# ray-project/ray_shuffling_data_loader

Hardware: AMD Instinct MI355X
Metric: shuffled_rows_per_sec (higher is better)
Workload: dtype bf16; 1 GPU; model=shuffling-data-loader + TabularMLP(100-512-256-128-1), global_batch=250000, rows_per_gpu=12500000, num_cols=100, batch_size_per_rank=250000, num_reducers=4, max_concurrent_epochs=2, parallelism=dp1, seed=0, burn_steps=0

## Files before the change

csrc/shuffle_kernels.hip:

```cpp

#include <hip/hip_runtime.h>
#include <hip/hip_fp16.h>
#include <hip/hip_bf16.h>

#include <cstdint>

#define RSDL_MAX_COLS 128

namespace rsdl {

__global__ void gather_rows_u4_kernel(
    const uint4* __restrict__ src,
    uint4* __restrict__ dst,
    const int64_t* __restrict__ perm,
    int64_t n_rows,
    int64_t row_u4) {
  const int64_t total = n_rows * row_u4;
  const int64_t stride = (int64_t)gridDim.x * blockDim.x;
  for (int64_t i = (int64_t)blockIdx.x * blockDim.x + threadIdx.x; i < total;
       i += stride) {
    const int64_t row = i / row_u4;
    const int64_t j = i - row * row_u4;
    dst[i] = src[perm[row] * row_u4 + j];
  }
// ... 28 lines not shown

struct ColDesc {
  int64_t col_ptr;
  int32_t packed_off;
  int32_t src_dtype;
  int32_t dst_dtype;
  int32_t numel;
};

struct ColTable {
  ColDesc cols[RSDL_MAX_COLS];
};

template <typename S, typename D>
__device__ __forceinline__ D cast_elem(S v) {
  return (D)v;
}
template <>
__device__ __forceinline__ __hip_bfloat16 cast_elem(float v) {
  return __float2bfloat16(v);
}
template <>
__device__ __forceinline__ __hip_bfloat16 cast_elem(double v) {
  return __float2bfloat16((float)v);
}
template <>
__device__ __forceinline__ __hip_bfloat16 cast_elem(int32_t v) {
  return __float2bfloat16((float)v);
}
template <>
__device__ __forceinline__ __hip_bfloat16 cast_elem(int64_t v) {
  return __float2bfloat16((float)v);
}
template <>
__device__ __forceinline__ float cast_elem(__hip_bfloat16 v) {
  return __bfloat162float(v);
}
template <>
__device__ __forceinline__ double cast_elem(__hip_bfloat16 v) {
  return (double)__bfloat162float(v);
}

__device__ __forceinline__ void unpack_vec4_f32_f32(
    const uint8_t* __restrict__ packed, int64_t row_stride,
    const int64_t* __restrict__ perm, float* __restrict__ dst,
    int32_t packed_off, int32_t numel, int64_t n_rows, int64_t tid,
    int64_t nthreads) {
// ... 57 lines not shown
}

template <typename S, typename D>
__device__ void pack_col_loop(
    uint8_t* __restrict__ packed,
    int64_t row_stride,
    const int64_t* __restrict__ perm,
    const S* __restrict__ src,
    int32_t packed_off,
    int32_t numel,
    int64_t n_rows,
    int64_t tid,
    int64_t nthreads) {
  const int64_t total = n_rows * numel;
  for (int64_t i = tid; i < total; i += nthreads) {
    const int64_t row = i / numel;
    const int64_t e = i - row * numel;
    const int64_t drow = perm ? perm[row] : row;
    D* dp = reinterpret_cast<D*>(packed + drow * row_stride + packed_off);
    dp[e] = cast_elem<S, D>(src[i]);
  }
}

#define RSDL_DISPATCH_DST(S_CTYPE, SRC_DT, DST_DT, CALL)                   \
  switch (DST_DT) {                                                        \
    case DT_F32: { using D = float; CALL; break; }                         \
    case DT_F64: { using D = double; CALL; break; }                        \
    case DT_I32: { using D = int32_t; CALL; break; }                       \
    case DT_I64: { using D = int64_t; CALL; break; }                       \
    case DT_BF16: { using D = __hip_bfloat16; CALL; break; }               \
    default: break;                                                        \
  }

#define RSDL_DISPATCH_PAIR(SRC_DT, DST_DT, CALL)                           \
  switch (SRC_DT) {                                                        \
    case DT_F32: { using S = float; RSDL_DISPATCH_DST(float, SRC_DT,       \
                   DST_DT, CALL); break; }                                 \
    case DT_F64: { using S = double; RSDL_DISPATCH_DST(double, SRC_DT,     \
                   DST_DT, CALL); break; }                                 \
    case DT_I32: { using S = int32_t; RSDL_DISPATCH_DST(int32_t, SRC_DT,   \
                   DST_DT, CALL); break; }                                 \
    case DT_I64: { using S = int64_t; RSDL_DISPATCH_DST(int64_t, SRC_DT,   \
                   DST_DT, CALL); break; }                                 \
    default: break;                                                        \
  }

// ... 4 lines not shown
    ColTable table,
    int32_t num_cols,
    int64_t n_rows) {
  const int32_t c = blockIdx.y;
  if (c >= num_cols) return;
  const ColDesc d = table.cols[c];
  const int64_t tid = (int64_t)blockIdx.x * blockDim.x + threadIdx.x;
  const int64_t nthreads = (int64_t)gridDim.x * blockDim.x;
  if (d.src_dtype == DT_F32 && (d.numel & 3) == 0 &&
      (d.packed_off & 15) == 0) {
    if (d.dst_dtype == DT_F32) {
      unpack_vec4_f32_f32(packed, row_stride, perm,
                          reinterpret_cast<float*>(d.col_ptr), d.packed_off,
                          d.numel, n_rows, tid, nthreads);
      return;
    }
    if (d.dst_dtype == DT_BF16) {
      unpack_vec4_f32_bf16(packed, row_stride, perm,
                           reinterpret_cast<__hip_bfloat16*>(d.col_ptr),
                           d.packed_off, d.numel, n_rows, tid, nthreads);
      return;
    }
  }
  RSDL_DISPATCH_PAIR(
      d.src_dtype, d.dst_dtype,
      (unpack_col_loop<S, D>(packed, row_stride, perm,
                             reinterpret_cast<D*>(d.col_ptr), d.packed_off,
                             d.numel, n_rows, tid, nthreads)));
}

__global__ void pack_columns_kernel(
    uint8_t* __restrict__ packed,
    int64_t row_stride,
    const int64_t* __restrict__ perm,
    ColTable table,
    int32_t num_cols,
    int64_t n_rows) {
  const int32_t c = blockIdx.y;
  if (c >= num_cols) return;
  const ColDesc d = table.cols[c];
  const int64_t tid = (int64_t)blockIdx.x * blockDim.x + threadIdx.x;
  const int64_t nthreads = (int64_t)gridDim.x * blockDim.x;
  RSDL_DISPATCH_PAIR(
      d.dst_dtype, d.src_dtype,
      (pack_col_loop<S, D>(packed, row_stride, perm,
                           reinterpret_cast<const S*>(d.col_ptr),
                           d.packed_off, d.numel, n_rows, tid, nthreads)));
}


#define RSDL_PART_MAX_DESTS 1024
// ... 523 lines not shown
  const ColDesc d = table.cols[c];
  const int64_t tid = (int64_t)blockIdx.x * blockDim.x + threadIdx.x;
  const int64_t nthreads = (int64_t)gridDim.x * blockDim.x;
  const bool al16 =
      ((reinterpret_cast<uintptr_t>(packed) + (uintptr_t)d.packed_off) &
       15) == 0;
  const int32_t ab = abase.base[c];
  if (ab < 0) {
    if (d.src_dtype == DT_F32 && (d.numel & 3) == 0 &&
        (d.packed_off & 15) == 0) {
      if (d.dst_dtype == DT_F32) {
        unpack_vec4_f32_f32(packed, row_stride, perm,
                            reinterpret_cast<float*>(d.col_ptr),
                            d.packed_off, d.numel, n_rows, tid, nthreads);
        return;
      }
      if (d.dst_dtype == DT_BF16) {
        unpack_vec4_f32_bf16(packed, row_stride, perm,
                             reinterpret_cast<__hip_bfloat16*>(d.col_ptr),
                             d.packed_off, d.numel, n_rows, tid, nthreads);
        return;
      }
    }
    RSDL_DISPATCH_PAIR(
        d.src_dtype, d.dst_dtype,
        (unpack_col_loop<S, D>(packed, row_stride, perm,
                               reinterpret_cast<D*>(d.col_ptr),
                               d.packed_off, d.numel, n_rows, tid,
                               nthreads)));
    return;
  }
  const double2* aff = aff_table + ab;
  const bool fill = has_fill != 0;
  const bool vec_dst = d.dst_dtype == DT_F32 || d.dst_dtype == DT_BF16;
  if (vec_dst && (d.numel & 3) == 0 && d.src_dtype == DT_F64) {
    if (d.dst_dtype == DT_BF16) {
      __hip_bfloat16* o = reinterpret_cast<__hip_bfloat16*>(d.col_ptr);
      if (al16)
        unpack_affine_vec4_f64<__hip_bfloat16, true>(
            packed, row_stride, perm, o, aff, d.packed_off, d.numel, n_rows,
            tid, nthreads, fill, fill_f);
      else
        unpack_affine_vec4_f64<__hip_bfloat16, false>(
            packed, row_stride, perm, o, aff, d.packed_off, d.numel, n_rows,
            tid, nthreads, fill, fill_f);
    } else {
// ... 9 lines not shown
    }
    return;
  }
  if (vec_dst && (d.numel & 3) == 0 && d.src_dtype == DT_F32 && al16) {
    if (d.dst_dtype == DT_BF16)
      unpack_affine_vec4_f32<__hip_bfloat16>(
          packed, row_stride, perm,
          reinterpret_cast<__hip_bfloat16*>(d.col_ptr), aff, d.packed_off,
          d.numel, n_rows, tid, nthreads, fill, fill_f);
    else
      unpack_affine_vec4_f32<float>(
          packed, row_stride, perm, reinterpret_cast<float*>(d.col_ptr),
          aff, d.packed_off, d.numel, n_rows, tid, nthreads, fill, fill_f);
    return;
  }
  RSDL_DISPATCH_PAIR(
      d.src_dtype, d.dst_dtype,
      (unpack_affine_col_loop<S, D>(packed, row_stride, perm,
                                    reinterpret_cast<D*>(d.col_ptr), aff,
                                    d.packed_off, d.numel, n_rows, tid,
                                    nthreads, fill, fill_f)));
}

void launch_column_stats(
    const void* packed, int64_t row_stride, int64_t n_rows,
    const StatsTable& table, int32_t num_cols, int32_t total_elems,
    int32_t num_blocks, int64_t* part_n, double* part_s, double* part_ss,
    double* pivot, int64_t* out_n, double* out_s, double* out_ss,
    hipStream_t stream) {
  hipLaunchKernelGGL(column_stats_kernel, dim3(num_blocks),
                     dim3(RSDL_STATS_THREADS), 0, stream,
                     reinterpret_cast<const uint8_t*>(packed), row_stride,
                     n_rows, table, num_cols, total_elems, part_n, part_s,
                     part_ss, pivot);
  const int threads = 64;
  hipLaunchKernelGGL(column_stats_combine_kernel,
                     dim3((total_elems + threads - 1) / threads),
                     dim3(threads), 0, stream, part_n, part_s, part_ss,
                     num_blocks, total_elems, out_n, out_s, out_ss);
}

void launch_unpack_permute_affine(
    const void* packed, int64_t row_stride, const int64_t* perm,
    const ColTable& table, const AffineBase& abase, const void* aff_table,
    int32_t num_cols, int64_t n_rows, int32_t has_fill, float fill_f,
    hipStream_t stream) {
// ... 14 lines not shown
```

csrc/shuffle_ops.cpp:

```cpp

#include <torch/extension.h>

#include <c10/hip/HIPStream.h>
#include <hip/hip_runtime.h>

#include <cmath>
#include <cstdlib>
#include <cstring>
#include <tuple>
#include <vector>

#include "chain.h"
#include "step_glue.h"

namespace rsdl {

enum DType : int32_t {
  DT_F32 = 0,
  DT_F64 = 1,
  DT_I32 = 2,
  DT_I64 = 3,
  DT_F16 = 4,
  DT_BF16 = 5,
  DT_U8 = 6,
// ... 30 lines not shown
  int32_t elem_base;
};

struct StatsTable {
  StatsCol cols[128];
};

struct AffineBase {
  int32_t base[128];
};

void launch_column_stats(const void* packed, int64_t row_stride,
                         int64_t n_rows, const StatsTable& table,
                         int32_t num_cols, int32_t total_elems,
                         int32_t num_blocks, int64_t* part_n, double* part_s,
                         double* part_ss, double* pivot, int64_t* out_n,
                         double* out_s, double* out_ss, hipStream_t stream);
void launch_unpack_permute_affine(const void* packed, int64_t row_stride,
                                  const int64_t* perm, const ColTable& table,
                                  const AffineBase& abase,
                                  const void* aff_table, int32_t num_cols,
                                  int64_t n_rows, int32_t has_fill,
                                  float fill_f, hipStream_t stream);
void launch_partition_hist(const int32_t* dest, int32_t* block_counts,
                           int64_t n, int32_t num_dests, int32_t num_blocks,
                           hipStream_t stream);
void launch_partition_scatter(const int32_t* dest, const int32_t* block_base,
                              int32_t* perm_out, int64_t n, int32_t num_dests,
                              int32_t num_blocks, hipStream_t stream);
void launch_pack_tiled(void* packed, int64_t row_stride, const ColTable& table,
                       int32_t num_cols, int64_t n_rows, int32_t tile_rows,
                       int64_t lds_bytes, int32_t n8, hipStream_t stream);
void launch_wgrad_bf16(const void* dy, const void* x, float* dW, float* db,
                       int64_t M, int32_t N, int32_t K, int32_t split_m,
                       hipStream_t stream);
void launch_wgrad_wide(const void* dy, const void* x, float* dW, float* db,
                       int64_t M, int32_t N, int32_t K, int32_t split_m,
                       hipStream_t stream);
void launch_relu_bwd_bias(const void* dy, const void* y, void* dx,
                          float* db_part, int64_t nvec, int32_t N,
                          int32_t grid, hipStream_t stream);

namespace {

int32_t dtype_code(at::ScalarType st) {
  switch (st) {
// ... 159 lines not shown
    TORCH_CHECK(o.size(0) == n_rows, "output rows mismatch");
    const int64_t numel = o.numel() / n_rows;
    const int64_t esz = src_elem_bytes(src_dtype_codes[c]);
    TORCH_CHECK(packed_offsets[c] >= 0 && packed_offsets[c] % esz == 0 &&
                    packed_offsets[c] + numel * esz <= stride,
                "column ", c, " does not fit the packed row");
    TORCH_CHECK(aff_base[c] < 0 ||
                    aff_base[c] + numel <= aff_table.size(0),
                "affine table too short for column ", c);
    table.cols[c] = ColDesc{
        reinterpret_cast<int64_t>(o.data_ptr()),
        (int32_t)packed_offsets[c],
        (int32_t)src_dtype_codes[c],
        dtype_code(o.scalar_type()),
        (int32_t)numel,
    };
    abase.base[c] = aff_base[c] < 0 ? -1 : (int32_t)aff_base[c];
  }
  launch_unpack_permute_affine(
      packed.data_ptr(), stride, perm_ptr, table, abase,
      aff_table.data_ptr(), (int32_t)outs.size(), n_rows,
      nan_fill.has_value() ? 1 : 0,
      nan_fill.has_value() ? (float)*nan_fill : 0.0f, current_stream());
}

std::vector<at::Tensor> column_stats(
    const at::Tensor& packed, const std::vector<int64_t>& packed_offsets,
    const std::vector<int64_t>& src_dtype_codes,
    const std::vector<int64_t>& numels) {
  TORCH_CHECK(packed.is_cuda(), "packed must be on GPU");
  TORCH_CHECK(packed.scalar_type() == at::kByte && packed.dim() == 2 &&
                  packed.is_contiguous(),
              "packed must be contiguous uint8 [rows, row_stride]");
  TORCH_CHECK(packed_offsets.size() == src_dtype_codes.size() &&
                  packed_offsets.size() == numels.size(),
              "descriptor length mismatch");
  TORCH_CHECK(!numels.empty() && numels.size() <= 128,
              "1..128 columns per launch");
  const int64_t n_rows = packed.size(0);
  const int64_t stride = packed.size(1);
  TORCH_CHECK(n_rows > 0, "column_stats needs at least one row");
  StatsTable table{};
  int64_t total = 0;
  for (size_t c = 0; c < numels.size(); ++c) {
    const int64_t esz = src_elem_bytes(src_dtype_codes[c]);
    TORCH_CHECK(numels[c] >= 1 && packed_offsets[c] >= 0 &&
// ... 975 lines not shown
              wide ? 6 : 5, "] on part's GPU");
  TORCH_CHECK(M >= 0, "eval_accumulate: M must not be negative");
  launch_eval_accumulate(part.data_ptr<float>(), part.size(0), M,
                         acc.data_ptr<double>(), wide ? 5 : 4,
                         current_stream());
}

}

PYBIND11_MODULE(TORCH_EXTENSION_NAME, m) {
  m.doc() = "MI355X (gfx950) fused shuffle kernels";
  m.def("gather_rows", &rsdl::gather_rows, "row gather of packed rows",
        py::arg("src"), py::arg("perm"));
  m.def("gather_rows_out", &rsdl::gather_rows_out, py::arg("src"),
        py::arg("perm"), py::arg("dst"));
  m.def("unpack_permute", &rsdl::unpack_permute, py::arg("packed"),
        py::arg("perm"), py::arg("outs"), py::arg("packed_offsets"),
        py::arg("src_dtype_codes"));
  m.def("unpack_permute_affine", &rsdl::unpack_permute_affine,
        py::arg("packed"), py::arg("perm"), py::arg("outs"),
        py::arg("packed_offsets"), py::arg("src_dtype_codes"),
        py::arg("aff_table"), py::arg("aff_base"),
        py::arg("nan_fill") = c10::nullopt);
  m.def("column_stats", &rsdl::column_stats, py::arg("packed"),
        py::arg("packed_offsets"), py::arg("src_dtype_codes"),
        py::arg("numels"));
  m.def("pack_columns", &rsdl::pack_columns, py::arg("cols"),
        py::arg("packed_offsets"), py::arg("packed_dtype_codes"),
        py::arg("row_stride"), py::arg("perm") = c10::nullopt);
  m.def("pack_columns_tiled", &rsdl::pack_columns_tiled, py::arg("cols"),
        py::arg("packed_offsets"), py::arg("packed_dtype_codes"),
        py::arg("row_stride"), py::arg("out") = c10::nullopt);
  m.def("partition_build_perm", &rsdl::partition_build_perm, py::arg("dest"),
        py::arg("num_dests"));
  m.def("wgrad_bf16", &rsdl::wgrad_bf16, py::arg("dy"), py::arg("x"),
        py::arg("with_bias") = true);
  m.def("relu_bwd_bias", &rsdl::relu_bwd_bias, py::arg("dy"), py::arg("y"));
  m.def("swizzle_xt_bf16", &rsdl::swizzle_xt_bf16, py::arg("x"),
        py::arg("pi16") = false);
  m.def("wgrad_frag_bf16", &rsdl::wgrad_frag_bf16, py::arg("AT"),
        py::arg("BT"), py::arg("N"), py::arg("K"), py::arg("mchunks"),
        py::arg("nt_w"), py::arg("kt_w"), py::arg("variant") = 0);
  m.def("wgrad_frag_partials_bf16", &rsdl::wgrad_frag_partials_bf16,
        py::arg("AT"), py::arg("BT"), py::arg("N"), py::arg("K"),
        py::arg("mchunks"), py::arg("nt_w"), py::arg("kt_w"),
        py::arg("variant") = 0);
// ... 42 lines not shown
```

ray_shuffling_data_loader_amd/engine.py:

```python

import contextlib
import os
import sys
import threading
import time
from typing import Dict, List, Optional, Sequence, Tuple, Union

_VERBOSE = os.environ.get("RSDL_VERBOSE") == "1"


def _vlog(msg: str) -> None:
    if _VERBOSE:
        print(f"[rsdl-engine] {msg}", file=sys.stderr, flush=True)

import numpy as np
import torch

from ray_shuffling_data_loader_amd.io import (
    fuse_schema,
    infer_schema,
    read_files_packed,
)
from ray_shuffling_data_loader_amd.ops.shuffle_ops import (
    ColumnStats,
    column_stats,
    gather_rows,
    make_affine_table,
    merge_column_stats,
    partition_rows,
    stats_to_affine,
    unpack_permute,
)
from ray_shuffling_data_loader_amd.parallel import fabric
from ray_shuffling_data_loader_amd.utils.rowblock import RowBlock
from ray_shuffling_data_loader_amd.utils.schema import (
    Schema,
    dtype_bytes,
    homogeneous_dtype,
)


class ShuffleEngineFailure:

    __slots__ = ("error",)

    def __init__(self, error: BaseException):
        self.error = error


class ShuffleEngine:
    def __init__(
# ... 72 lines not shown
        probs = np.array(self.reducers_per_trainer, dtype=np.float64)
        probs /= probs.sum()
        self._dest_uniform = len(set(self.reducers_per_trainer)) == 1
        self._dest_cum = torch.from_numpy(np.cumsum(probs)).to(
            self.device, torch.float32
        )

        if schema is None:
            if not self.filenames:
                raise ValueError("need filenames or an explicit schema")
            schema = infer_schema(self.filenames[0])
        self.base_schema = schema
        self.out_schema = fuse_schema(schema, feature_matrix)

        if seed is None:
            seed = int(time.time_ns() % (2**31))
        self.seed = seed
        if self.device.type == "cuda":
            self._gen = torch.Generator(device=self.device)
        else:
            self._gen = torch.Generator()

        self._cached_source: Optional[torch.Tensor] = None
        self._stream = (
            torch.cuda.Stream(device=self.device)
            if self.device.type == "cuda"
            else None
        )
        self._thread: Optional[threading.Thread] = None
        self._error: Optional[BaseException] = None
        self.duration: Optional[float] = None

        self.normalize = normalize
        self.nan_fill = nan_fill
        self._stats_ready = threading.Event()
        self._col_stats: Optional[Dict[str, ColumnStats]] = None
        self._affine = None
        self._norm_names: List[str] = []
        if normalize is None:
            if nan_fill is not None:
                raise ValueError("nan_fill needs normalize")
        else:
            self._init_normalize(normalize)


    _NORM_DTYPES = (torch.float32, torch.float64, torch.int32, torch.int64)
# ... 120 lines not shown
        return dict(self._col_stats)


    def _get_source(self, epoch: int) -> torch.Tensor:
        if self._cached_source is not None:
            src = self._cached_source
            if src.device != self.device:
                src = src.to(self.device, non_blocking=True)
            return src
        if self.stats:
            for _ in self.my_files:
                self.stats.map_start(epoch)
        t0 = time.perf_counter()
        src = read_files_packed(
            self.my_files, self.base_schema, self.device, self.reader_threads
        )
        read_dur = time.perf_counter() - t0
        if self.stats:
            per_file = read_dur / max(1, len(self.my_files))
            for _ in self.my_files:
                self.stats.map_done(epoch, per_file, per_file)
        if self.normalize is not None and self._affine is None:
            self._fit(src)
        if self.source_cache in ("auto", "device"):
            self._cached_source = src
        elif self.source_cache == "host":
            if src.device.type == "cuda":
                host = torch.empty(
                    src.shape, dtype=src.dtype, pin_memory=True
                )
                host.copy_(src)
                self._cached_source = host
            else:
                self._cached_source = src
        return src


    def _sample_dest(self, n: int) -> torch.Tensor:
        if self._dest_uniform:
            return torch.randint(
                self.num_trainers,
                (n,),
                device=self.device,
                generator=self._gen,
                dtype=torch.long,
            )
        u = torch.rand(n, device=self.device, generator=self._gen)
        return torch.searchsorted(self._dest_cum, u, right=True).clamp_(
            max=self.num_trainers - 1
        )

    def _make_partition(
        self, rows: torch.Tensor, idx: torch.Tensor
    ) -> RowBlock:
        schema = self.out_schema
        hom = homogeneous_dtype(schema)
        use_views = (
            not self.out_dtypes
            and self.normalize is None
            and (
                self.output == "views"
                or (self.output == "auto" and hom is not None)
            )
        )
        if use_views and hom is not None:
            esz = dtype_bytes(hom)
            gathered = gather_rows(rows, idx)
            typed = gathered.view(hom)
            cols: Dict[str, torch.Tensor] = {}
            for spec in schema.columns:
                o = schema.offsets[spec.name] // esz
                if spec.numel == 1:
                    cols[spec.name] = typed[:, o]
                else:
                    cols[spec.name] = typed[:, o : o + spec.numel]
            return RowBlock(cols)
        if self._affine is not None:
            cols = unpack_permute(
                rows,
                schema,
                perm=idx.to(torch.long),
                out_dtypes=self.out_dtypes,
                affine=self._affine,
                nan_fill=self.nan_fill,
            )
            return RowBlock(cols)
        cols = unpack_permute(
# ... 142 lines not shown
```

ray_shuffling_data_loader_amd/ops/__init__.py:

```python
from ray_shuffling_data_loader_amd.ops.shuffle_ops import (
    gather_rows,
    pack_columns,
    partition_rows,
    relu_mask_words,
    t_frag_swizzle,
    t_frag_unswizzle,
    unpack_permute,
    wgrad,
    wgrad_frag,
)
```

ray_shuffling_data_loader_amd/ops/shuffle_ops.py:

```python

from typing import Dict, List, NamedTuple, Optional, Sequence, Tuple, Union

import os

import numpy as np
import torch

from ray_shuffling_data_loader_amd.utils.schema import (
    Schema,
    TORCH_TO_NUMPY_DTYPE,
)

_hip = None
_hip_err = None


def _load_hip():
    global _hip, _hip_err
    if _hip is None and _hip_err is None:
        try:
            from ray_shuffling_data_loader_amd import _rsdl_hip

            _hip = _rsdl_hip
        except ImportError as e:
            _hip_err = e
    if _hip is None:
        raise RuntimeError(
            "ray_shuffling_data_loader_amd._rsdl_hip extension is not built "
            "but a GPU tensor was passed to a shuffle op. Build it with "
            "`python setup.py build_ext --inplace` (PYTORCH_ROCM_ARCH="
            f"gfx950). Original import error: {_hip_err}"
# ... 118 lines not shown
        spec = schema.col(name)
        pair = []
        for t in (shift, scale):
            t = torch.as_tensor(t, dtype=torch.float64).detach().cpu()
            t = t.reshape(-1)
            if t.numel() == 1 and spec.numel > 1:
                t = t.expand(spec.numel)
            if t.numel() != spec.numel:
                raise ValueError(
                    f"affine entry for column {name!r} needs {spec.numel} "
                    f"elements, got {t.numel()}"
                )
            pair.append(t.contiguous())
        entries[name] = (pair[0], pair[1])
        base[name] = n_elems
        n_elems += spec.numel
        rows.append(torch.stack(pair, dim=1))
    table = None
    if device is not None and torch.device(device).type == "cuda":
        table = torch.cat(rows).contiguous().to(device)
    return AffineTable(entries, base, table)


def unpack_permute(
    packed: torch.Tensor,
    schema: Schema,
    perm: Optional[torch.Tensor] = None,
    out_dtypes: Optional[Dict[str, torch.dtype]] = None,
    affine: Union[
        None, AffineTable, Dict[str, Tuple[torch.Tensor, torch.Tensor]]
    ] = None,
    nan_fill: Optional[float] = None,
) -> Dict[str, torch.Tensor]:
    out_dtypes = out_dtypes or {}
    n = perm.numel() if perm is not None else packed.shape[0]
    if affine is not None and not isinstance(affine, AffineTable):
        affine = make_affine_table(affine, schema, packed.device)
    if affine is not None and not affine.entries:
        affine = None
    if packed.is_cuda:
        hip = _load_hip()
        outs, offs, codes = [], [], []
        result: Dict[str, torch.Tensor] = {}
        for spec in schema.columns:
            dst_dt = out_dtypes.get(spec.name, spec.dtype)
            shape = (n,) if spec.numel == 1 else (n, spec.numel)
            o = torch.empty(shape, dtype=dst_dt, device=packed.device)
            outs.append(o)
            offs.append(schema.offsets[spec.name])
            codes.append(_dtype_code(spec.dtype))
            result[spec.name] = o
        if affine is None:
            hip.unpack_permute(packed, perm, outs, offs, codes)
            return result
        table = affine.table
        if table is None or table.device != packed.device:
            table = make_affine_table(
                affine.entries, schema, packed.device
            ).table
        bases = [affine.base.get(spec.name, -1) for spec in schema.columns]
        hip.unpack_permute_affine(
            packed, perm, outs, offs, codes, table, bases, nan_fill
        )
        return result
    packed_np = packed.numpy()
    perm_np = perm.cpu().numpy() if perm is not None else None
    result = {}
    for spec in schema.columns:
        np_dt = TORCH_TO_NUMPY_DTYPE[spec.dtype]
        view = _np_strided_view(packed_np, schema, spec.name, spec.numel, np_dt)
        arr = view[perm_np] if perm_np is not None else np.ascontiguousarray(
            view
        )
        t = torch.from_numpy(arr)
        dst_dt = out_dtypes.get(spec.name, spec.dtype)
        if affine is not None and spec.name in affine.entries:
            shift, scale = affine.entries[spec.name]
            x = t.double()
            y = ((x - shift) * scale).float()
            if nan_fill is not None:
                y = torch.where(
                    torch.isnan(x),
                    torch.tensor(float(nan_fill), dtype=torch.float64)
                    .float(),
                    y,
                )
            t = y.to(dst_dt)
        elif dst_dt != spec.dtype:
            t = t.to(dst_dt)
        if spec.numel == 1:
            t = t.reshape(n)
        result[spec.name] = t
    return result




class ColumnStats(NamedTuple):

    count: torch.Tensor
    mean: torch.Tensor
    std: torch.Tensor


_STATS_DTYPES = (torch.float32, torch.float64, torch.int32, torch.int64)
_STATS_PIVOT_ROWS = 64


def _finish_stats(count, s, ss, pivot) -> ColumnStats:
    count = count.to(torch.int64)
    nz = count > 0
    cnt = count.clamp(min=1).double()
    dmean = s / cnt
    var = (ss / cnt - dmean * dmean).clamp_(min=0.0)
    zero = torch.zeros_like(dmean)
    mean = torch.where(nz, pivot + dmean, zero)
# ... 222 lines not shown
```

Before: 330.5 million rows/s.

## Narrow packed rows to output dtypes before shuffle and add row-sweep unpack

```diff
diff --git a/csrc/shuffle_kernels.hip b/csrc/shuffle_kernels.hip
--- a/csrc/shuffle_kernels.hip
+++ b/csrc/shuffle_kernels.hip
@@ -74,7 +74,7 @@
 }
 template <>
 __device__ __forceinline__ __hip_bfloat16 cast_elem(double v) {
-  return __float2bfloat16((float)v);
+  return __double2bfloat16(v);
 }
 template <>
 __device__ __forceinline__ __hip_bfloat16 cast_elem(int32_t v) {
@@ -178,6 +178,59 @@
   }
 }
 
+template <typename V>
+__device__ __forceinline__ void copy_col_loop(
+    const uint8_t* __restrict__ src, int64_t src_pitch,
+    const int64_t* __restrict__ perm, uint8_t* __restrict__ dst,
+    int64_t dst_pitch, int32_t col_bytes, int64_t n_rows, int64_t tid,
+    int64_t nthreads) {
+  const int32_t lanes = col_bytes / (int32_t)sizeof(V);
+  const int64_t total = n_rows * lanes;
+  for (int64_t i = tid; i < total; i += nthreads) {
+    const int64_t row = i / lanes;
+    const int64_t j = i - row * lanes;
+    const int64_t srow = perm ? perm[row] : row;
+    const V v = *reinterpret_cast<const V*>(
+        src + srow * src_pitch + j * (int64_t)sizeof(V));
+    *reinterpret_cast<V*>(dst + row * dst_pitch + j * (int64_t)sizeof(V)) = v;
+  }
+}
+
+__device__ __forceinline__ void copy_col(
+    const uint8_t* __restrict__ src, int64_t src_pitch,
+    const int64_t* __restrict__ perm, uint8_t* __restrict__ dst,
+    int64_t dst_pitch, int32_t col_bytes, int64_t n_rows, int64_t tid,
+    int64_t nthreads) {
+  const uintptr_t m = reinterpret_cast<uintptr_t>(src) |
+                      reinterpret_cast<uintptr_t>(dst) |
+                      (uintptr_t)src_pitch | (uintptr_t)dst_pitch |
+                      (uintptr_t)col_bytes;
+  if ((m & 15) == 0)
+    copy_col_loop<uint4>(src, src_pitch, perm, dst, dst_pitch, col_bytes,
+                         n_rows, tid, nthreads);
+  else if ((m & 7) == 0)
+    copy_col_loop<uint2>(src, src_pitch, perm, dst, dst_pitch, col_bytes,
+                         n_rows, tid, nthreads);
+  else if ((m & 3) == 0)
+    copy_col_loop<uint32_t>(src, src_pitch, perm, dst, dst_pitch, col_bytes,
+                            n_rows, tid, nthreads);
+  else if ((m & 1) == 0)
+    copy_col_loop<uint16_t>(src, src_pitch, perm, dst, dst_pitch, col_bytes,
+                            n_rows, tid, nthreads);
+  else
+    copy_col_loop<uint8_t>(src, src_pitch, perm, dst, dst_pitch, col_bytes,
+                           n_rows, tid, nthreads);
+}
+
+__device__ __forceinline__ int32_t dtype_size(int32_t dt) {
+  switch (dt) {
+    case DT_F64: case DT_I64: return 8;
+    case DT_F32: case DT_I32: return 4;
+    case DT_F16: case DT_BF16: return 2;
+    default: return 1;
+  }
+}
+
 #define RSDL_DISPATCH_DST(S_CTYPE, SRC_DT, DST_DT, CALL)                   \
   switch (DST_DT) {                                                        \
     case DT_F32: { using D = float; CALL; break; }                         \
@@ -228,11 +281,59 @@
       return;
     }
   }
+  if (d.src_dtype == d.dst_dtype) {
+    const int32_t col_bytes = d.numel * dtype_size(d.src_dtype);
+    copy_col(packed + d.packed_off, row_stride, perm,
+             reinterpret_cast<uint8_t*>(d.col_ptr), col_bytes, col_bytes,
+             n_rows, tid, nthreads);
+    return;
+  }
   RSDL_DISPATCH_PAIR(
       d.src_dtype, d.dst_dtype,
       (unpack_col_loop<S, D>(packed, row_stride, perm,
                              reinterpret_cast<D*>(d.col_ptr), d.packed_off,
                              d.numel, n_rows, tid, nthreads)));
+}
+
+#define RSDL_SWEEP_MAX_COLS 8
+
+struct SweepCol {
+  int64_t col_ptr;
+  int32_t lane0;
+  int32_t lanes;
+};
+
+struct SweepTable {
+  SweepCol cols[RSDL_SWEEP_MAX_COLS];
+};
+
+__global__ void unpack_rows_sweep_kernel(
+    const uint2* __restrict__ packed,
+    int64_t row_u2,
+    const int64_t* __restrict__ perm,
+    SweepTable table,
+    int32_t num_cols,
+    int32_t lanes_per_row,
+    int64_t n_rows) {
+  const int64_t total = n_rows * lanes_per_row;
+  const int64_t stride = (int64_t)gridDim.x * blockDim.x;
+  for (int64_t i = (int64_t)blockIdx.x * blockDim.x + threadIdx.x; i < total;
+       i += stride) {
+    const int64_t row = i / lanes_per_row;
+    const int32_t j = (int32_t)(i - row * lanes_per_row);
+    const int64_t srow = perm ? perm[row] : row;
+#pragma unroll
+    for (int32_t c = 0; c < RSDL_SWEEP_MAX_COLS; ++c) {
+      if (c < num_cols) {
+        const SweepCol d = table.cols[c];
+        const int32_t k = j - d.lane0;
+        if ((uint32_t)k < (uint32_t)d.lanes) {
+          reinterpret_cast<uint2*>(d.col_ptr)[row * d.lanes + k] =
+              packed[srow * row_u2 + j];
+        }
+      }
+    }
+  }
 }
 
 __global__ void pack_columns_kernel(
@@ -802,6 +903,13 @@
         return;
       }
     }
+    if (d.src_dtype == d.dst_dtype) {
+      const int32_t col_bytes = d.numel * dtype_size(d.src_dtype);
+      copy_col(packed + d.packed_off, row_stride, perm,
+               reinterpret_cast<uint8_t*>(d.col_ptr), col_bytes, col_bytes,
+               n_rows, tid, nthreads);
+      return;
+    }
     RSDL_DISPATCH_PAIR(
         d.src_dtype, d.dst_dtype,
         (unpack_col_loop<S, D>(packed, row_stride, perm,
@@ -857,6 +965,226 @@
                                     nthreads, fill, fill_f)));
 }
 
+
+struct NarrowCol {
+  int32_t src_off;
+  int32_t dst_off;
+  int32_t src_dtype;
+  int32_t dst_dtype;
+  int32_t numel;
+  int32_t aff_base;
+};
+
+struct NarrowTable {
+  NarrowCol cols[RSDL_MAX_COLS];
+};
+
+template <typename S, bool WIDE>
+__device__ __forceinline__ void load4(const uint8_t* __restrict__ sp,
+                                      S (&x)[4]) {
+  if constexpr (sizeof(S) == 8) {
+    if constexpr (WIDE) {
+      const double2 v0 = reinterpret_cast<const double2*>(sp)[0];
+      const double2 v1 = reinterpret_cast<const double2*>(sp)[1];
+      x[0] = v0.x; x[1] = v0.y; x[2] = v1.x; x[3] = v1.y;
+    } else {
+      const double* dp = reinterpret_cast<const double*>(sp);
+      x[0] = dp[0]; x[1] = dp[1]; x[2] = dp[2]; x[3] = dp[3];
+    }
+  } else {
+    if constexpr (WIDE) {
+      const float4 v = *reinterpret_cast<const float4*>(sp);
+      x[0] = v.x; x[1] = v.y; x[2] = v.z; x[3] = v.w;
+    } else {
+      const float2 v0 = reinterpret_cast<const float2*>(sp)[0];
+      const float2 v1 = reinterpret_cast<const float2*>(sp)[1];
+      x[0] = v0.x; x[1] = v0.y; x[2] = v1.x; x[3] = v1.y;
+    }
+  }
+}
+
+template <typename S, typename D, bool WIDE, bool AFF>
+__device__ __forceinline__ void narrow_vec4_loop(
+    const uint8_t* __restrict__ src, int64_t src_stride,
+    uint8_t* __restrict__ dst, int64_t dst_stride,
+    const double2* __restrict__ aff, int32_t numel, int64_t n_rows,
+    int64_t tid, int64_t nthreads, bool fill, float fill_f) {
+  const int32_t groups = numel >> 2;
+  const int64_t total = n_rows * groups;
+  for (int64_t i = tid; i < total; i += nthreads) {
+    const int64_t row = i / groups;
+    const int64_t g = i - row * groups;
+    S x[4];
+    load4<S, WIDE>(src + row * src_stride + g * (int64_t)(4 * sizeof(S)), x);
+    D* dp = reinterpret_cast<D*>(dst + row * dst_stride) + (g << 2);
+    if constexpr (AFF) {
+      const double2* ap = aff + (g << 2);
+      store4<D>(dp, affine_f32((double)x[0], ap[0], fill, fill_f),
+                affine_f32((double)x[1], ap[1], fill, fill_f),
+                affine_f32((double)x[2], ap[2], fill, fill_f),
+                affine_f32((double)x[3], ap[3], fill, fill_f));
+    } else {
+      union {
+        D h[4];
+        uint32_t u[sizeof(D)];
+      } o;
+#pragma unroll
+      for (int32_t k = 0; k < 4; ++k) o.h[k] = cast_elem<S, D>(x[k]);
+      if constexpr (sizeof(D) == 2)
+        *reinterpret_cast<uint2*>(dp) = make_uint2(o.u[0], o.u[1]);
+      else
+        *reinterpret_cast<uint4*>(dp) =
+            make_uint4(o.u[0], o.u[1], o.u[2], o.u[3]);
+    }
+  }
+}
+
+template <typename S, typename D>
+__device__ __forceinline__ void narrow_vec4(
+    const uint8_t* __restrict__ src, int64_t src_stride,
+    uint8_t* __restrict__ dst, int64_t dst_stride,
+    const double2* __restrict__ aff, int32_t numel, int64_t n_rows,
+    int64_t tid, int64_t nthreads, bool fill, float fill_f, bool wide) {
+  if (aff != nullptr) {
+    if (wide)
+      narrow_vec4_loop<S, D, true, true>(src, src_stride, dst, dst_stride,
+                                         aff, numel, n_rows, tid, nthreads,
+                                         fill, fill_f);
+    else
+      narrow_vec4_loop<S, D, false, true>(src, src_stride, dst, dst_stride,
+                                          aff, numel, n_rows, tid, nthreads,
+                                          fill, fill_f);
+  } else {
+    if (wide)
+      narrow_vec4_loop<S, D, true, false>(src, src_stride, dst, dst_stride,
+                                          aff, numel, n_rows, tid, nthreads,
+                                          fill, fill_f);
+    else
+      narrow_vec4_loop<S, D, false, false>(src, src_stride, dst, dst_stride,
+                                           aff, numel, n_rows, tid, nthreads,
+                                           fill, fill_f);
+  }
+}
+
+template <typename S, typename D>
+__device__ void narrow_col_loop(
+    const uint8_t* __restrict__ src, int64_t src_stride,
+    uint8_t* __restrict__ dst, int64_t dst_stride,
+    const double2* __restrict__ aff, int32_t numel, int64_t n_rows,
+    int64_t tid, int64_t nthreads, bool fill, float fill_f) {
+  const int64_t total = n_rows * numel;
+  for (int64_t i = tid; i < total; i += nthreads) {
+    const int64_t row = i / numel;
+    const int64_t e = i - row * numel;
+    const S x = reinterpret_cast<const S*>(src + row * src_stride)[e];
+    D* dp = reinterpret_cast<D*>(dst + row * dst_stride);
+    if (aff != nullptr)
+      dp[e] = cast_elem<float, D>(
+          affine_f32((double)x, aff[e], fill, fill_f));
+    else
+      dp[e] = cast_elem<S, D>(x);
+  }
+}
+
+__global__ void narrow_rows_kernel(
+    const uint8_t* __restrict__ src,
+    int64_t src_stride,
+    uint8_t* __restrict__ dst,
+    int64_t dst_stride,
+    NarrowTable table,
+    const double2* __restrict__ aff_table,
+    int32_t num_cols,
+    int64_t n_rows,
+    int32_t has_fill,
+    float fill_f,
+    int32_t pad_off) {
+  const int32_t c = blockIdx.y;
+  const int64_t tid = (int64_t)blockIdx.x * blockDim.x + threadIdx.x;
+  const int64_t nthreads = (int64_t)gridDim.x * blockDim.x;
+  if (c >= num_cols) {
+    const int32_t pad = (int32_t)dst_stride - pad_off;
+    const int64_t total = n_rows * pad;
+    for (int64_t i = tid; i < total; i += nthreads) {
+      const int64_t row = i / pad;
+      dst[row * dst_stride + pad_off + (i - row * pad)] = 0;
+    }
+    return;
+  }
+  const NarrowCol d = table.cols[c];
+  const uint8_t* sp = src + d.src_off;
+  uint8_t* dp = dst + d.dst_off;
+  if (d.src_dtype == d.dst_dtype && d.aff_base < 0) {
+    copy_col(sp, src_stride, nullptr, dp, dst_stride,
+             d.numel * dtype_size(d.src_dtype), n_rows, tid, nthreads);
+    return;
+  }
+  const double2* aff = d.aff_base < 0 ? nullptr : aff_table + d.aff_base;
+  const bool fill = has_fill != 0;
+  const uintptr_t sa = reinterpret_cast<uintptr_t>(sp);
+  const uintptr_t da = reinterpret_cast<uintptr_t>(dp);
+  const bool vec_src = (d.src_dtype == DT_F64 || d.src_dtype == DT_F32) &&
+                       (d.numel & 3) == 0 && (sa & 7) == 0;
+  const bool wide = (sa & 15) == 0;
+  if (vec_src && d.dst_dtype == DT_BF16 && (da & 7) == 0) {
+    if (d.src_dtype == DT_F64)
+      narrow_vec4<double, __hip_bfloat16>(sp, src_stride, dp, dst_stride, aff,
+                                          d.numel, n_rows, tid, nthreads,
+                                          fill, fill_f, wide);
+    else
+      narrow_vec4<float, __hip_bfloat16>(sp, src_stride, dp, dst_stride, aff,
+                                         d.numel, n_rows, tid, nthreads,
+                                         fill, fill_f, wide);
+    return;
+  }
+  if (vec_src && d.dst_dtype == DT_F32 && (da & 15) == 0) {
+    if (d.src_dtype == DT_F64)
+      narrow_vec4<double, float>(sp, src_stride, dp, dst_stride, aff,
+                                 d.numel, n_rows, tid, nthreads, fill,
+                                 fill_f, wide);
+    else
+      narrow_vec4<float, float>(sp, src_stride, dp, dst_stride, aff, d.numel,
+                                n_rows, tid, nthreads, fill, fill_f, wide);
+    return;
+  }
+  RSDL_DISPATCH_PAIR(
+      d.src_dtype, d.dst_dtype,
+      (narrow_col_loop<S, D>(sp, src_stride, dp, dst_stride, aff, d.numel,
+                             n_rows, tid, nthreads, fill, fill_f)));
+}
+
+void launch_narrow_rows(
+    const void* src, int64_t src_stride, void* dst, int64_t dst_stride,
+    const NarrowTable& table, const void* aff_table, int32_t num_cols,
+    int64_t n_rows, int32_t has_fill, float fill_f, int32_t pad_off,
+    hipStream_t stream) {
+  const int threads = 256;
+  int64_t bx = (n_rows + threads - 1) / threads;
+  if (bx > 4096) bx = 4096;
+  if (bx < 1) bx = 1;
+  dim3 grid((uint32_t)bx,
+            (uint32_t)(num_cols + (pad_off < dst_stride ? 1 : 0)));
+  hipLaunchKernelGGL(narrow_rows_kernel, grid, dim3(threads), 0, stream,
+                     reinterpret_cast<const uint8_t*>(src), src_stride,
+                     reinterpret_cast<uint8_t*>(dst), dst_stride, table,
+                     reinterpret_cast<const double2*>(aff_table), num_cols,
+                     n_rows, has_fill, fill_f, pad_off);
+}
+
+void launch_unpack_rows_sweep(
+    const void* packed, int64_t row_stride, const int64_t* perm,
+    const SweepTable& table, int32_t num_cols, int32_t lanes_per_row,
+    int64_t n_rows, hipStream_t stream) {
+  const int64_t total = n_rows * lanes_per_row;
+  const int threads = 256;
+  int64_t blocks = (total + threads - 1) / threads;
+  if (blocks > 65535 * 16) blocks = 65535 * 16;
+  if (blocks < 1) blocks = 1;
+  hipLaunchKernelGGL(unpack_rows_sweep_kernel, dim3((uint32_t)blocks),
+                     dim3(threads), 0, stream,
+                     reinterpret_cast<const uint2*>(packed), row_stride / 8,
+                     perm, table, num_cols, lanes_per_row, n_rows);
+}
+
 void launch_column_stats(
     const void* packed, int64_t row_stride, int64_t n_rows,
     const StatsTable& table, int32_t num_cols, int32_t total_elems,
diff --git a/csrc/shuffle_ops.cpp b/csrc/shuffle_ops.cpp
--- a/csrc/shuffle_ops.cpp
+++ b/csrc/shuffle_ops.cpp
@@ -76,6 +76,38 @@
                                   const void* aff_table, int32_t num_cols,
                                   int64_t n_rows, int32_t has_fill,
                                   float fill_f, hipStream_t stream);
+struct NarrowCol {
+  int32_t src_off;
+  int32_t dst_off;
+  int32_t src_dtype;
+  int32_t dst_dtype;
+  int32_t numel;
+  int32_t aff_base;
+};
+
+struct NarrowTable {
+  NarrowCol cols[128];
+};
+
+struct SweepCol {
+  int64_t col_ptr;
+  int32_t lane0;
+  int32_t lanes;
+};
+
+struct SweepTable {
+  SweepCol cols[8];
+};
+
+void launch_narrow_rows(const void* src, int64_t src_stride, void* dst,
+                        int64_t dst_stride, const NarrowTable& table,
+                        const void* aff_table, int32_t num_cols,
+                        int64_t n_rows, int32_t has_fill, float fill_f,
+                        int32_t pad_off, hipStream_t stream);
+void launch_unpack_rows_sweep(const void* packed, int64_t row_stride,
+                              const int64_t* perm, const SweepTable& table,
+                              int32_t num_cols, int32_t lanes_per_row,
+                              int64_t n_rows, hipStream_t stream);
 void launch_partition_hist(const int32_t* dest, int32_t* block_counts,
                            int64_t n, int32_t num_dests, int32_t num_blocks,
                            hipStream_t stream);
@@ -281,6 +313,147 @@
       aff_table.data_ptr(), (int32_t)outs.size(), n_rows,
       nan_fill.has_value() ? 1 : 0,
       nan_fill.has_value() ? (float)*nan_fill : 0.0f, current_stream());
+}
+
+int64_t any_elem_bytes(int64_t code) {
+  switch (code) {
+    case DT_F64: case DT_I64: return 8;
+    case DT_F32: case DT_I32: return 4;
+    case DT_F16: case DT_BF16: return 2;
+    case DT_U8: return 1;
+    default:
+      TORCH_CHECK(false, "unsupported packed dtype code ", code);
+  }
+}
+
+at::Tensor narrow_rows(const at::Tensor& packed, int64_t dst_stride,
+                       int64_t pad_off,
+                       const std::vector<int64_t>& src_offsets,
+                       const std::vector<int64_t>& src_codes,
+                       const std::vector<int64_t>& dst_offsets,
+                       const std::vector<int64_t>& dst_codes,
+                       const std::vector<int64_t>& numels,
+                       const c10::optional<at::Tensor>& aff_table,
+                       const std::vector<int64_t>& aff_base,
+                       const c10::optional<double>& nan_fill) {
+  TORCH_CHECK(packed.is_cuda(), "packed must be on GPU");
+  TORCH_CHECK(packed.scalar_type() == at::kByte && packed.dim() == 2 &&
+                  packed.is_contiguous(),
+              "packed must be contiguous uint8 [rows, row_stride]");
+  const size_t nc = numels.size();
+  TORCH_CHECK(src_offsets.size() == nc && src_codes.size() == nc &&
+                  dst_offsets.size() == nc && dst_codes.size() == nc &&
+                  aff_base.size() == nc,
+              "descriptor length mismatch");
+  TORCH_CHECK(nc >= 1 && nc <= 128, "1..128 columns per launch");
+  const int64_t n_rows = packed.size(0);
+  const int64_t src_stride = packed.size(1);
+  TORCH_CHECK(src_stride % 16 == 0 && dst_stride > 0 && dst_stride % 16 == 0,
+              "row strides must be multiples of 16");
+  TORCH_CHECK(pad_off >= 0 && pad_off <= dst_stride,
+              "pad_off outside the narrow row");
+  int64_t aff_rows = 0;
+  if (aff_table.has_value()) {
+    TORCH_CHECK(aff_table->is_cuda() &&
+                    aff_table->scalar_type() == at::kDouble &&
+                    aff_table->is_contiguous() && aff_table->dim() == 2 &&
+                    aff_table->size(1) == 2,
+                "aff_table must be contiguous float64 [elems, 2] on GPU");
+    aff_rows = aff_table->size(0);
+  }
+  NarrowTable table{};
+  for (size_t c = 0; c < nc; ++c) {
+    const int64_t ssz = any_elem_bytes(src_codes[c]);
+    const int64_t dsz = any_elem_bytes(dst_codes[c]);
+    const bool same = src_codes[c] == dst_codes[c] && aff_base[c] < 0;
+    if (!same) {
+      TORCH_CHECK(src_codes[c] == DT_F32 || src_codes[c] == DT_F64 ||
+                      src_codes[c] == DT_I32 || src_codes[c] == DT_I64,
+                  "column ", c, ": unsupported source dtype for a cast");
+      TORCH_CHECK(dst_codes[c] == DT_F32 || dst_codes[c] == DT_F64 ||
+                      dst_codes[c] == DT_I32 || dst_codes[c] == DT_I64 ||
+                      dst_codes[c] == DT_BF16,
+                  "column ", c, ": unsupported destination dtype for a cast");
+    }
+    TORCH_CHECK(numels[c] >= 1 && src_offsets[c] >= 0 &&
+                    src_offsets[c] % ssz == 0 &&
+                    src_offsets[c] + numels[c] * ssz <= src_stride,
+                "column ", c, " does not fit the wide row");
+    TORCH_CHECK(dst_offsets[c] >= 0 && dst_offsets[c] % dsz == 0 &&
+                    dst_offsets[c] + numels[c] * dsz <= pad_off,
+                "column ", c, " does not fit the narrow row");
+    TORCH_CHECK(aff_base[c] < 0 || aff_base[c] + numels[c] <= aff_rows,
+                "affine table too short for column ", c);
+    table.cols[c] = NarrowCol{
+        (int32_t)src_offsets[c], (int32_t)dst_offsets[c],
+        (int32_t)src_codes[c],   (int32_t)dst_codes[c],
+        (int32_t)numels[c],      aff_base[c] < 0 ? -1 : (int32_t)aff_base[c],
+    };
+  }
+  auto out = at::empty({n_rows, dst_stride}, packed.options());
+  if (n_rows == 0) return out;
+  launch_narrow_rows(packed.data_ptr(), src_stride, out.data_ptr(),
+                     dst_stride, table,
+                     aff_table.has_value() ? aff_table->data_ptr() : nullptr,
+                     (int32_t)nc, n_rows, nan_fill.has_value() ? 1 : 0,
+                     nan_fill.has_value() ? (float)*nan_fill : 0.0f,
+                     (int32_t)pad_off, current_stream());
+  return out;
+}
+
+void unpack_permute_sweep(const at::Tensor& packed,
+                          const c10::optional<at::Tensor>& perm,
+                          const std::vector<at::Tensor>& outs,
+                          const std::vector<int64_t>& packed_offsets,
+                          const std::vector<int64_t>& src_dtype_codes) {
+  TORCH_CHECK(packed.is_cuda(), "packed must be on GPU");
+  TORCH_CHECK(packed.scalar_type() == at::kByte && packed.dim() == 2 &&
+                  packed.is_contiguous(),
+              "packed must be contiguous uint8 [rows, row_stride]");
+  TORCH_CHECK(outs.size() == packed_offsets.size() &&
+                  outs.size() == src_dtype_codes.size(),
+              "descriptor length mismatch");
+  TORCH_CHECK(outs.size() >= 1 && outs.size() <= 8,
+              "1..8 columns per sweep");
+  const int64_t stride = packed.size(1);
+  TORCH_CHECK(stride % 8 == 0 &&
+                  reinterpret_cast<uintptr_t>(packed.data_ptr()) % 8 == 0,
+              "packed rows must be 8-B aligned");
+  int64_t n_rows;
+  const int64_t* perm_ptr = nullptr;
+  if (perm.has_value()) {
+    TORCH_CHECK(perm->is_cuda() && perm->scalar_type() == at::kLong &&
+                    perm->is_contiguous(),
+                "perm must be contiguous int64 on GPU");
+    n_rows = perm->numel();
+    perm_ptr = perm->data_ptr<int64_t>();
+  } else {
+    n_rows = packed.size(0);
+  }
+  if (n_rows == 0) return;
+  SweepTable table{};
+  int64_t lanes_per_row = 0;
+  for (size_t c = 0; c < outs.size(); ++c) {
+    const auto& o = outs[c];
+    TORCH_CHECK(o.is_cuda() && o.is_contiguous(),
+                "output column must be contiguous GPU tensor");
+    TORCH_CHECK(o.size(0) == n_rows, "output rows mismatch");
+    TORCH_CHECK(dtype_code(o.scalar_type()) == src_dtype_codes[c],
+                "sweep: column ", c, " changes dtype");
+    const int64_t bytes =
+        o.numel() / n_rows * any_elem_bytes(src_dtype_codes[c]);
+    TORCH_CHECK(packed_offsets[c] >= 0 && packed_offsets[c] % 8 == 0 &&
+                    bytes % 8 == 0 && packed_offsets[c] + bytes <= stride &&
+                    reinterpret_cast<uintptr_t>(o.data_ptr()) % 8 == 0,
+                "sweep: column ", c, " is not made of whole 8-B lanes");
+    table.cols[c] = SweepCol{reinterpret_cast<int64_t>(o.data_ptr()),
+                             (int32_t)(packed_offsets[c] / 8),
+                             (int32_t)(bytes / 8)};
+    lanes_per_row = std::max(lanes_per_row, (packed_offsets[c] + bytes) / 8);
+  }
+  launch_unpack_rows_sweep(packed.data_ptr(), stride, perm_ptr, table,
+                           (int32_t)outs.size(), (int32_t)lanes_per_row,
+                           n_rows, current_stream());
 }
 
 std::vector<at::Tensor> column_stats(
@@ -1302,6 +1475,16 @@
         py::arg("packed_offsets"), py::arg("src_dtype_codes"),
         py::arg("aff_table"), py::arg("aff_base"),
         py::arg("nan_fill") = c10::nullopt);
+  m.def("narrow_rows", &rsdl::narrow_rows, py::arg("packed"),
+        py::arg("dst_stride"), py::arg("pad_off"), py::arg("src_offsets"),
+        py::arg("src_dtype_codes"), py::arg("dst_offsets"),
+        py::arg("dst_dtype_codes"), py::arg("numels"),
+        py::arg("aff_table") = c10::nullopt,
+        py::arg("aff_base") = std::vector<int64_t>(),
+        py::arg("nan_fill") = c10::nullopt);
+  m.def("unpack_permute_sweep", &rsdl::unpack_permute_sweep,
+        py::arg("packed"), py::arg("perm"), py::arg("outs"),
+        py::arg("packed_offsets"), py::arg("src_dtype_codes"));
   m.def("column_stats", &rsdl::column_stats, py::arg("packed"),
         py::arg("packed_offsets"), py::arg("src_dtype_codes"),
         py::arg("numels"));
diff --git a/ray_shuffling_data_loader_amd/engine.py b/ray_shuffling_data_loader_amd/engine.py
--- a/ray_shuffling_data_loader_amd/engine.py
+++ b/ray_shuffling_data_loader_amd/engine.py
@@ -27,6 +27,9 @@
     gather_rows,
     make_affine_table,
     merge_column_stats,
+    narrow_rows,
+    narrow_schema,
+    narrow_supported,
     partition_rows,
     stats_to_affine,
     unpack_permute,
@@ -145,6 +148,9 @@
             self._gen = torch.Generator()
 
         self._cached_source: Optional[torch.Tensor] = None
+        self._narrow_on = os.environ.get("RSDL_NARROW_CACHE", "1") != "0"
+        self._narrow_sweep = os.environ.get("RSDL_NARROW_SWEEP", "0") == "1"
+        self._narrow_schema: Optional[Schema] = None
         self._stream = (
             torch.cuda.Stream(device=self.device)
             if self.device.type == "cuda"
@@ -311,6 +317,23 @@
                 self.stats.map_done(epoch, per_file, per_file)
         if self.normalize is not None and self._affine is None:
             self._fit(src)
+        plan = self._narrow_plan()
+        if plan is not None:
+            src = narrow_rows(
+                src,
+                self.out_schema,
+                plan,
+                affine=self._affine,
+                nan_fill=self.nan_fill,
+            )
+            self._narrow_schema = plan
+            if src.device.type == "cuda":
+                torch.cuda.current_stream(src.device).synchronize()
+                torch.cuda.empty_cache()
+            _vlog(
+                f"rank {self.rank}: narrowed the source block "
+                f"{self.base_schema.row_stride} -> {plan.row_stride} B/row"
+            )
         if self.source_cache in ("auto", "device"):
             self._cached_source = src
         elif self.source_cache == "host":
@@ -323,6 +346,33 @@
             else:
                 self._cached_source = src
         return src
+
+    def _use_views(self) -> bool:
+        hom = homogeneous_dtype(self.out_schema)
+        return (
+            not self.out_dtypes
+            and self.normalize is None
+            and (
+                self.output == "views"
+                or (self.output == "auto" and hom is not None)
+            )
+        )
+
+    def _narrow_plan(self) -> Optional[Schema]:
+        if (
+            not self._narrow_on
+            or self._narrow_schema is not None
+            or self.source_cache not in ("auto", "device", "host")
+            or self._use_views()
+        ):
+            return None
+        plan = narrow_schema(self.out_schema, self.out_dtypes)
+        aff = tuple(self._affine.entries) if self._affine is not None else ()
+        if not narrow_supported(self.out_schema, plan, aff):
+            return None
+        if plan.row_stride >= self.base_schema.row_stride:
+            return None
+        return plan
 
 
     def _sample_dest(self, n: int) -> torch.Tensor:
@@ -342,16 +392,17 @@
     def _make_partition(
         self, rows: torch.Tensor, idx: torch.Tensor
     ) -> RowBlock:
+        if self._narrow_schema is not None:
+            cols = unpack_permute(
+                rows,
+                self._narrow_schema,
+                perm=idx.to(torch.long),
+                row_sweep=self._narrow_sweep,
+            )
+            return RowBlock(cols)
         schema = self.out_schema
         hom = homogeneous_dtype(schema)
-        use_views = (
-            not self.out_dtypes
-            and self.normalize is None
-            and (
-                self.output == "views"
-                or (self.output == "auto" and hom is not None)
-            )
-        )
+        use_views = self._use_views()
         if use_views and hom is not None:
             esz = dtype_bytes(hom)
             gathered = gather_rows(rows, idx)
diff --git a/ray_shuffling_data_loader_amd/ops/__init__.py b/ray_shuffling_data_loader_amd/ops/__init__.py
--- a/ray_shuffling_data_loader_amd/ops/__init__.py
+++ b/ray_shuffling_data_loader_amd/ops/__init__.py
@@ -1,5 +1,7 @@
 from ray_shuffling_data_loader_amd.ops.shuffle_ops import (
     gather_rows,
+    narrow_rows,
+    narrow_schema,
     pack_columns,
     partition_rows,
     relu_mask_words,
diff --git a/ray_shuffling_data_loader_amd/ops/shuffle_ops.py b/ray_shuffling_data_loader_amd/ops/shuffle_ops.py
--- a/ray_shuffling_data_loader_amd/ops/shuffle_ops.py
+++ b/ray_shuffling_data_loader_amd/ops/shuffle_ops.py
@@ -7,6 +7,7 @@
 import torch
 
 from ray_shuffling_data_loader_amd.utils.schema import (
+    ColumnSpec,
     Schema,
     TORCH_TO_NUMPY_DTYPE,
 )
@@ -171,6 +172,34 @@
     return AffineTable(entries, base, table)
 
 
+def _np_storage_dtype(dtype: torch.dtype):
+    if dtype == torch.bfloat16:
+        return np.dtype(np.int16)
+    return TORCH_TO_NUMPY_DTYPE[dtype]
+
+
+def _f64_to_bf16(t: torch.Tensor) -> torch.Tensor:
+    f = t.float()
+    back = f.double()
+    fi = f.view(torch.int32)
+    inexact = (back != t) & ~torch.isnan(t)
+    even = (fi & 1) == 0
+    one = torch.ones((), dtype=torch.int32)
+    step = torch.where(t.abs() > back.abs(), one, -one)
+    fi = torch.where(inexact & even, fi + step, fi)
+    return fi.view(torch.float32).to(torch.bfloat16)
+
+
+_SWEEP_MAX_COLS = 8
+
+
+def row_sweep_ok(schema: Schema) -> bool:
+    return 1 <= len(schema.columns) <= _SWEEP_MAX_COLS and all(
+        schema.offsets[c.name] % 8 == 0 and c.row_bytes % 8 == 0
+        for c in schema.columns
+    )
+
+
 def unpack_permute(
     packed: torch.Tensor,
     schema: Schema,
@@ -180,6 +209,7 @@
         None, AffineTable, Dict[str, Tuple[torch.Tensor, torch.Tensor]]
     ] = None,
     nan_fill: Optional[float] = None,
+    row_sweep: bool = False,
 ) -> Dict[str, torch.Tensor]:
     out_dtypes = out_dtypes or {}
     n = perm.numel() if perm is not None else packed.shape[0]
@@ -200,6 +230,16 @@
             codes.append(_dtype_code(spec.dtype))
             result[spec.name] = o
         if affine is None:
+            if (
+                row_sweep
+                and row_sweep_ok(schema)
+                and all(
+                    o.dtype == spec.dtype
+                    for o, spec in zip(outs, schema.columns)
+                )
+            ):
+                hip.unpack_permute_sweep(packed, perm, outs, offs, codes)
+                return result
             hip.unpack_permute(packed, perm, outs, offs, codes)
             return result
         table = affine.table
@@ -216,12 +256,14 @@
     perm_np = perm.cpu().numpy() if perm is not None else None
     result = {}
     for spec in schema.columns:
-        np_dt = TORCH_TO_NUMPY_DTYPE[spec.dtype]
+        np_dt = _np_storage_dtype(spec.dtype)
         view = _np_strided_view(packed_np, schema, spec.name, spec.numel, np_dt)
         arr = view[perm_np] if perm_np is not None else np.ascontiguousarray(
             view
         )
         t = torch.from_numpy(arr)
+        if t.dtype != spec.dtype:
+            t = t.view(spec.dtype)
         dst_dt = out_dtypes.get(spec.name, spec.dtype)
         if affine is not None and spec.name in affine.entries:
             shift, scale = affine.entries[spec.name]
@@ -236,11 +278,107 @@
                 )
             t = y.to(dst_dt)
         elif dst_dt != spec.dtype:
-            t = t.to(dst_dt)
+            if spec.dtype == torch.float64 and dst_dt == torch.bfloat16:
+                t = _f64_to_bf16(t)
+            else:
+                t = t.to(dst_dt)
         if spec.numel == 1:
             t = t.reshape(n)
         result[spec.name] = t
     return result
+
+
+
+_CAST_SRC_DTYPES = (torch.float32, torch.float64, torch.int32, torch.int64)
+_CAST_DST_DTYPES = _CAST_SRC_DTYPES + (torch.bfloat16,)
+
+
+def narrow_schema(
+    schema: Schema, out_dtypes: Optional[Dict[str, torch.dtype]] = None
+) -> Schema:
+    out_dtypes = out_dtypes or {}
+    return Schema(
+        [
+            ColumnSpec(c.name, out_dtypes.get(c.name, c.dtype), c.numel)
+            for c in schema.columns
+        ]
+    )
+
+
+def narrow_supported(
+    schema: Schema, narrow: Schema, affine_names: Sequence[str] = ()
+) -> bool:
+    for spec in schema.columns:
+        dst = narrow.col(spec.name).dtype
+        if spec.dtype == dst and spec.name not in affine_names:
+            continue
+        if spec.dtype not in _CAST_SRC_DTYPES or dst not in _CAST_DST_DTYPES:
+            return False
+    return True
+
+
+def narrow_rows(
+    packed: torch.Tensor,
+    schema: Schema,
+    narrow: Schema,
+    affine: Union[
+        None, AffineTable, Dict[str, Tuple[torch.Tensor, torch.Tensor]]
+    ] = None,
+    nan_fill: Optional[float] = None,
+) -> torch.Tensor:
+    if affine is not None and not isinstance(affine, AffineTable):
+        affine = make_affine_table(affine, schema, packed.device)
+    if affine is not None and not affine.entries:
+        affine = None
+    aff_names = tuple(affine.entries) if affine is not None else ()
+    if [c.name for c in narrow.columns] != schema.names:
+        raise ValueError("narrow schema must list the same columns")
+    if not narrow_supported(schema, narrow, aff_names):
+        raise TypeError("narrow_rows: unsupported column dtype pair")
+    n = packed.shape[0]
+    if packed.is_cuda:
+        hip = _load_hip()
+        table = None
+        if affine is not None:
+            table = affine.table
+            if table is None or table.device != packed.device:
+                table = make_affine_table(
+                    affine.entries, schema, packed.device
+                ).table
+        return hip.narrow_rows(
+            packed,
+            narrow.row_stride,
+            narrow.payload_bytes,
+            [schema.offsets[c.name] for c in schema.columns],
+            [_dtype_code(c.dtype) for c in schema.columns],
+            [narrow.offsets[c.name] for c in schema.columns],
+            [_dtype_code(narrow.col(c.name).dtype) for c in schema.columns],
+            [c.numel for c in schema.columns],
+            table,
+            [
+                affine.base.get(c.name, -1) if affine is not None else -1
+                for c in schema.columns
+            ],
+            nan_fill,
+        )
+    cols = unpack_permute(
+        packed,
+        schema,
+        None,
+        out_dtypes={c.name: c.dtype for c in narrow.columns},
+        affine=affine,
+        nan_fill=nan_fill,
+    )
+    out = torch.zeros(n, narrow.row_stride, dtype=torch.uint8)
+    out_np = out.numpy()
+    for spec in narrow.columns:
+        np_dt = _np_storage_dtype(spec.dtype)
+        view = _np_strided_view(out_np, narrow, spec.name, spec.numel, np_dt)
+        t = cols[spec.name].reshape(n, spec.numel).contiguous()
+        if spec.dtype == torch.bfloat16:
+            t = t.view(torch.int16)
+        view[:] = t.numpy()
+    return out
 
 
 
```

Result: faster. 347.5 million rows/s (median of 6 runs) (+5.2%).
